# alexklwong/calibrated-backprojection-network

Hardware: AMD Instinct MI355X
Metric: depth-completion frames/sec at 352x1216 (higher is better)
Workload: dtype f32; 1 GPU; KITTI 352x1216, batch 32/GPU, fp32, full KBNet forward in HIP, random xavier weights; frames_per_gpu=32, global_batch=32, height=352, width=1216, n_ranks_seen=1, collective_backend=nccl, gathered_frames=32, launch=HIP graph replay, 2 concurrent sub-batch branch(es)

## Files before the change

calibrated-backprojection-network_amd/csrc/conv1x1s2_split.hip:

```cpp

#include "split_common.h"

namespace kbn {

template <int N, int NBX>
__device__ __forceinline__ void c1_wait_b(f32x4 (&b)[NBX][2]) {
    static_assert(NBX == 1, "one 32-filter block per wave (the 4 x 2 wave form with two was measured and removed)");
    asm volatile("s_waitcnt vmcnt(%2)" : "+v"(b[0][0]), "+v"(b[0][1]) : "n"(N));
}
template <int N>
__device__ __forceinline__ void c1_wait_a(float (&v)[8]) {
    asm volatile("s_waitcnt vmcnt(%8)" : "+v"(v[0]), "+v"(v[1]), "+v"(v[2]), "+v"(v[3]), "+v"(v[4]), "+v"(v[5]), "+v"(v[6]), "+v"(v[7]) : "n"(N));
}

template <int RG, int NB, bool ONE = false>
__global__ __launch_bounds__(SP_THREADS, 1) void conv1x1s2_split_kernel(const SplitConvParams p) {
    constexpr int TH = 8, MB = TH / RG, NT = 128, NPIX = TH * SP_TW;
    static_assert(32 * NB * (8 / RG) == NT, "128 filters per workgroup");
    constexpr int A_PART = 2 * NPIX * 16, A_BYTES = 2 * A_PART;
    constexpr int B_CHUNK = 2 * 2 * NT * 16;
    extern __shared__ __attribute__((aligned(16))) unsigned char smem[];
    asm volatile("s_setreg_imm32_b32 hwreg(HW_REG_MODE, 6, 2), 0");
    const int tid = threadIdx.x, lane = tid & 63;
    const int wave = __builtin_amdgcn_readfirstlane(tid >> 6);
    const int rg = wave % RG, fg = wave / RG;
    const int lm = lane & 31, g = lane >> 5;
    int bid = xcd_remap(blockIdx.x, p.nblocks);
    const int nt = bid % p.nTilesN;
    bid /= p.nTilesN;
    const int tx = bid % p.tilesX;
    bid /= p.tilesX;
    const int ty = bid % p.tilesY;
    const int n = bid / p.tilesY;
    const int oy0 = ty * TH, ox0 = tx * SP_TW;
    const int H = p.H, W = p.W, sH = p.sH, sW = p.sW;
    const long long plane = (long long)sH * sW;
    const int nchunks = p.Cin / SP_CK, last = nchunks - 1;
    float prescale, unscale;
    sp_act_scale(p, n, prescale, unscale);

    const int kg_st = wave >> 2, t256 = tid & 255;
    const int sy = 2 * (oy0 + (t256 >> 5)), sx = 2 * (ox0 + (t256 & 31));
    const int goff = (sy < sH && sx < sW) ? (sy * sW + sx) * 4 : -1;
    const int goff_sub = goff >= 0 ? ((sy >> 1) * W + (sx >> 1)) * 4 : -1;
    const long long plane_sub = (long long)H * W;
    const unsigned char* wp_nt = reinterpret_cast<const unsigned char*>(p.wp) + (long long)nt * nchunks * B_CHUNK;

    float va[2][8];
    auto load_chunk = [&](float (&v)[8], int chunk) {
        int c = chunk * SP_CK, s = 0;
        if (p.nsrc > 1 && c >= p.srcC[0]) { c -= p.srcC[0]; s = 1; }
        const bool sub = p.sub0 && s == 0;
        const long long pl = sub ? plane_sub : plane;
        const float* base = p.src[s] + (long long)n * p.src_bstride[s] + (long long)(c + kg_st * 8) * pl;
        const int go = sub ? goff_sub : goff;
        const unsigned voff = go < 0 ? 0u : (unsigned)go;
#pragma unroll
        for (int k = 0; k < 8; ++k) {
            const float* sb = base + (long long)k * pl;
            asm volatile("global_load_dword %0, %1, %2" : "=v"(v[k]) : "v"(voff), "s"(sb) : "memory");
        }
    };
    auto store_chunk = [&](int buf, const float (&vin)[8]) {
        unsigned char* A = smem + buf * A_BYTES + kg_st * NPIX * 16;
        float v[8];
#pragma unroll
        for (int k = 0; k < 8; ++k) v[k] = goff >= 0 ? vin[k] : 0.f;
        sph8 h1, h2;
        sp_split8(v, prescale, h1, h2);
        *reinterpret_cast<sph8*>(A + t256 * 16) = h1;
        *reinterpret_cast<sph8*>(A + A_PART + t256 * 16) = h2;
    };
    const unsigned boff = (unsigned)((g * NT + fg * 32 * NB + lm) * 16);
    auto load_b = [&](f32x4 (&b)[NB][2], int chunk) {
        const unsigned char* base = wp_nt + (long long)chunk * B_CHUNK;
#pragma unroll
        for (int nb = 0; nb < NB; ++nb)
#pragma unroll
            for (int t = 0; t < 2; ++t) {
                const unsigned char* sb = base + (t * 2 * NT + nb * 32) * 16;
                asm volatile("global_load_dwordx4 %0, %1, %2" : "=v"(b[nb][t]) : "v"(boff), "s"(sb) : "memory");
            }
    };

    spf16 acc[MB][NB], lo[MB][NB];
#pragma unroll
    for (int mb = 0; mb < MB; ++mb)
#pragma unroll
        for (int nb = 0; nb < NB; ++nb)
#pragma unroll
            for (int i = 0; i < 16; ++i) { acc[mb][nb][i] = 0.f; lo[mb][nb][i] = 0.f; }

    const unsigned char* const aptr = smem + (g * NPIX + MB * rg * SP_TW + lm) * 16;
    f32x4 bq[2][NB][2];
    constexpr int NLB = 2 * NB, NLA = 8;
    auto body = [&](int c, auto par_tag) {
        constexpr int PAR = decltype(par_tag)::value;
        load_b(bq[PAR ^ 1], min(c + 1, last));
        load_chunk(va[PAR], min(c + 2, last));
        c1_wait_b<NLA + NLB + NLA>(bq[PAR]);
        if (c <= last) {
            sph8 bw[NB][2], a[MB][2];
#pragma unroll
            for (int nb = 0; nb < NB; ++nb) {
                bw[nb][0] = __builtin_bit_cast(sph8, bq[PAR][nb][0]);
                bw[nb][1] = __builtin_bit_cast(sph8, bq[PAR][nb][1]);
            }
            const int abuf = PAR * A_BYTES;
#pragma unroll
            for (int mb = 0; mb < MB; ++mb)
#pragma unroll
                for (int t = 0; t < 2; ++t) a[mb][t] = *reinterpret_cast<const sph8*>(aptr + abuf + t * A_PART + mb * SP_TW * 16);
            constexpr int TA[3] = {0, 0, 1}, TBP[3] = {0, 1, 0};
#pragma unroll
            for (int t = 0; t < (ONE ? 1 : 3); ++t)
#pragma unroll
                for (int mb = 0; mb < MB; ++mb)
#pragma unroll
                    for (int nb = 0; nb < NB; ++nb) {
                        spf16& d = t > 0 ? lo[mb][nb] : acc[mb][nb];
                        d = __builtin_amdgcn_mfma_f32_32x32x16_f16(a[mb][TA[t]], bw[nb][TBP[t]], d, 0, 0, 0);
                    }
        }
        c1_wait_a<NLB + NLA>(va[PAR ^ 1]);
        store_chunk(PAR ^ 1, va[PAR ^ 1]);
        __syncthreads();
    };

    load_chunk(va[0], 0);
    c1_wait_a<0>(va[0]);
    store_chunk(0, va[0]);
    load_b(bq[0], 0);
    load_chunk(va[1], min(1, last));
    __syncthreads();
    for (int c = 0; c < nchunks; c += 2) {
        body(c, std::integral_constant<int, 0>{});
        body(c + 1, std::integral_constant<int, 1>{});
    }
    asm volatile("s_waitcnt vmcnt(0)" ::: "memory");

    const long long oplane = (long long)H * W;
    float* outn = p.out + (long long)n * p.out_bstride;
    const float* xyzn = p.xyz ? p.xyz + (long long)n * p.xyz_bstride : nullptr;
    const float slope = p.act ? p.slope : 1.f;
    const bool vec4 = p.vec4 != 0;
    float amax = 0.f;
#pragma unroll
    for (int nb = 0; nb < NB; ++nb) {
        const int oc = nt * NT + fg * 32 * NB + nb * 32 + lm;
        const float inv = p.inv_scale[oc] * unscale;
        if (oc >= p.OC) continue;
        float wx[3] = {0.f, 0.f, 0.f};
        if (xyzn) { wx[0] = p.wxyz[oc * 3]; wx[1] = p.wxyz[oc * 3 + 1]; wx[2] = p.wxyz[oc * 3 + 2]; }
#pragma unroll
        for (int mb = 0; mb < MB; ++mb) {
            const int Y = oy0 + MB * rg + mb;
            if (Y >= H) continue;
            float* o = outn + (long long)oc * oplane + (long long)Y * W + ox0 + 4 * g;
#pragma unroll
            for (int q4 = 0; q4 < 4; ++q4) {
                const int X = ox0 + 8 * q4 + 4 * g;
                if (X >= W) continue;
                f32x4 v;
#pragma unroll
                for (int j = 0; j < 4; ++j) {
                    float t = __builtin_fmaf(lo[mb][nb][q4 * 4 + j], 0.00048828125f, acc[mb][nb][q4 * 4 + j]) * inv;
                    if (xyzn && X + j < W) {
                        const float* xp = xyzn + (long long)Y * W + X + j;
                        t += wx[0] * xp[0] + wx[1] * xp[oplane] + wx[2] * xp[2 * oplane];
                    }
                    v[j] = t > 0.f ? t : t * slope;
                }
                if (vec4) {
                    *reinterpret_cast<f32x4*>(o + 8 * q4) = v;
                    amax = sp_amax4(amax, v);
                } else {
#pragma unroll
                    for (int j = 0; j < 4; ++j)
                        if (X + j < W) { o[8 * q4 + j] = v[j]; amax = fmaxf(amax, fin_abs(v[j])); }
                }
            }
        }
    }
    if (p.out_amax) absmax_commit(p.out_amax + n, amax);
}

__global__ void kb_xyz_s2_kernel(const float* __restrict__ depth, long long dbs, int Cd, int H, int W, const float* __restrict__ proj,
                                 const float* __restrict__ kinv, int act, float slope, float* __restrict__ xyz, long long xbs,
                                 int oh, int ow) {
    const int idx = blockIdx.x * blockDim.x + threadIdx.x, n = blockIdx.y;
    if (idx >= oh * ow) return;
    const int oy = idx / ow, ox = idx - oy * ow;
    const int Y = 2 * oy, X = 2 * ox;
    const long long HW = (long long)H * W;
    const float* db = depth + (long long)n * dbs + (long long)Y * W + X;
    float a0 = 0.f, a1 = 0.f, a2 = 0.f, a3 = 0.f;
    int c = 0;
    for (; c + 3 < Cd; c += 4) {
        a0 = fmaf(proj[c], db[(long long)c * HW], a0);
        a1 = fmaf(proj[c + 1], db[(long long)(c + 1) * HW], a1);
        a2 = fmaf(proj[c + 2], db[(long long)(c + 2) * HW], a2);
        a3 = fmaf(proj[c + 3], db[(long long)(c + 3) * HW], a3);
    }
    for (; c < Cd; ++c) a0 = fmaf(proj[c], db[(long long)c * HW], a0);
    const float a = (a0 + a1) + (a2 + a3);
    const float z = act ? leaky_relu(a, slope) : a;
    const float* ki = kinv + (long long)n * 9;
    float* o = xyz + (long long)n * xbs + idx;
#pragma unroll
    for (int j = 0; j < 3; ++j)
        o[(long long)j * oh * ow] = (fmaf(ki[j * 3 + 1], (float)Y, ki[j * 3 + 0] * (float)X) + ki[j * 3 + 2]) * z;
}

__global__ void copy_wxyz_kernel(const float* __restrict__ w, float* __restrict__ wxyz, int OC, int cin_total, int xyz_offset) {
    const int e = blockIdx.x * blockDim.x + threadIdx.x;
    if (e < OC * 3) wxyz[e] = w[(long long)(e / 3) * cin_total + xyz_offset + e % 3];
}

}

extern "C" {

static size_t c1_panel_bytes(int out_channels, int cin) {
    return (size_t)kbn::ceil_div(out_channels, 128) * (128 * 4 + (size_t)(cin / kbn::SP_CK) * (2 * 2 * 128 * 16));
}

size_t kbn_conv1x1s2_split_packed_weight_bytes(int out_channels, int tensor_channels, int has_xyz) {
    if (out_channels < 1 || tensor_channels < 1 || (tensor_channels % kbn::SP_CK) != 0) return 0;
    return c1_panel_bytes(out_channels, tensor_channels) + (has_xyz ? (size_t)out_channels * 3 * 4 : 0);
}

int kbn_conv1x1s2_split_pack_weight(const float* weight, void* packed, int out_channels, int in_channels, int xyz_offset,
                                    kbn_stream_t stream) {
    using namespace kbn;
    const bool has_xyz = xyz_offset >= 0;
    const int cin = in_channels - (has_xyz ? 3 : 0);
    if (!weight || !packed || (has_xyz && xyz_offset > cin) || kbn_conv1x1s2_split_packed_weight_bytes(out_channels, cin, has_xyz) == 0)
        return KBN_ERR_INVALID_ARGUMENT;
    const int ocpad = ceil_div(out_channels, 128) * 128;
    float* inv = static_cast<float*>(packed);
    _Float16* wp = reinterpret_cast<_Float16*>(inv + ocpad);
    const long long total = (long long)((c1_panel_bytes(out_channels, cin) - (size_t)ocpad * 4) / 2);
    split_pack_launch(weight, inv, wp, out_channels, in_channels, cin, 128, total, 1, has_xyz ? xyz_offset : cin, has_xyz ? 3 : 0,
                      (hipStream_t)stream);
    if (has_xyz) {
        float* wxyz = reinterpret_cast<float*>(static_cast<unsigned char*>(packed) + c1_panel_bytes(out_channels, cin));
        hipLaunchKernelGGL(copy_wxyz_kernel, dim3(ceil_div(out_channels * 3, 256)), dim3(256), 0, (hipStream_t)stream, weight, wxyz,
                           out_channels, in_channels, xyz_offset);
    }
    KBN_CHECK_LAUNCH();
    return KBN_OK;
}

int kbn_conv1x1s2_split_forward(const kbn_conv_src* srcs, int n_src, const void* packed_weight, const float* xyz,
                                long long xyz_batch_stride, float* out, long long out_batch_stride, int n, int out_channels,
                                int height, int width, int act_exponent, int apply_activation, float negative_slope,
                                unsigned* out_absmax, kbn_stream_t stream) {
    using namespace kbn;
    if (act_exponent < -60 || act_exponent > 60) return KBN_ERR_INVALID_ARGUMENT;
    if (!srcs || n_src < 1 || n_src > 2 || !packed_weight || !out || n < 1 || out_channels < 1 || height < 1 || width < 1)
        return KBN_ERR_INVALID_ARGUMENT;
    if (knob(KNOB_NO_SPLIT)) return KBN_ERR_UNSUPPORTED;
    SplitConvParams p{};
    int cin = 0;
    for (int s = 0; s < n_src; ++s) {
        const kbn_conv_src& a = srcs[s];
        if (a.kind != KBN_SRC_TENSOR || !a.data || a.channels < 1 || (a.channels % SP_CK) != 0) return KBN_ERR_UNSUPPORTED;
        const bool sub = s == 0 && n_src == 2 && a.src_height == height && a.src_width == width &&
                         (srcs[1].src_height != height || srcs[1].src_width != width);
        if (sub) p.sub0 = 1;
        else {
            if (!p.sH) { p.sH = a.src_height; p.sW = a.src_width; }
            if (a.src_height != p.sH || a.src_width != p.sW) return KBN_ERR_INVALID_ARGUMENT;
        }
        p.src[s] = a.data; p.src_bstride[s] = a.batch_stride; p.srcC[s] = a.channels;
        cin += a.channels;
    }
    if (ceil_div(p.sH, 2) != height || ceil_div(p.sW, 2) != width) return KBN_ERR_INVALID_ARGUMENT;
    if ((long long)p.sH * p.sW > 0x1fffffffLL) return KBN_ERR_UNSUPPORTED;
    if (n_src == 1) { p.src[1] = p.src[0]; p.src_bstride[1] = p.src_bstride[0]; p.srcC[1] = 0; }
    p.nsrc = n_src;
    if (srcs[0].absmax && (n_src == 1 || srcs[1].absmax)) { p.amax[0] = srcs[0].absmax; p.amax[1] = n_src > 1 ? srcs[1].absmax : nullptr; }
    p.out_amax = out_absmax;
    p.nTilesN = ceil_div(out_channels, 128);
    p.inv_scale = static_cast<const float*>(packed_weight);
    p.wp = reinterpret_cast<const _Float16*>(p.inv_scale + p.nTilesN * 128);
    p.xyz = xyz; p.xyz_bstride = xyz_batch_stride;
    p.wxyz = xyz ? reinterpret_cast<const float*>(static_cast<const unsigned char*>(packed_weight) + c1_panel_bytes(out_channels, cin)) : nullptr;
    p.out = out; p.out_bstride = out_batch_stride;
    p.N = n; p.OC = out_channels; p.Cin = cin; p.H = height; p.W = width;
    p.tilesX = ceil_div(width, SP_TW); p.tilesY = ceil_div(height, 8);
    const long long blocks = (long long)p.tilesX * p.tilesY * n * p.nTilesN;
    if (blocks > 0x7fffffffLL) return KBN_ERR_UNSUPPORTED;
    p.nblocks = (int)blocks;
    p.act = apply_activation ? 1 : 0; p.slope = negative_slope;
    p.prescale = ldexpf(1.f, act_exponent); p.unscale = ldexpf(1.f, -act_exponent);
    p.vec4 = !((width & 3) || (reinterpret_cast<uintptr_t>(out) & 15) || (out_batch_stride & 3)) ? 1 : 0;
    if (knob(KNOB_FP16_ONE_TERM))
        hipLaunchKernelGGL((conv1x1s2_split_kernel<2, 1, true>), dim3(p.nblocks), dim3(SP_THREADS), 2 * 2 * 2 * 256 * 16, (hipStream_t)stream, p);
    else hipLaunchKernelGGL((conv1x1s2_split_kernel<2, 1>), dim3(p.nblocks), dim3(SP_THREADS), 2 * 2 * 2 * 256 * 16, (hipStream_t)stream, p);
    KBN_CHECK_LAUNCH();
    return KBN_OK;
}

int kbn_kb_xyz_s2_forward(const float* depth, long long depth_batch_stride, int depth_channels, int height, int width,
                          const float* proj_weight, const float* kinv, int apply_activation, float negative_slope, float* xyz,
                          long long xyz_batch_stride, int n, kbn_stream_t stream) {
    using namespace kbn;
    if (!depth || !proj_weight || !kinv || !xyz || n < 1 || depth_channels < 1 || height < 1 || width < 1) return KBN_ERR_INVALID_ARGUMENT;
    const int oh = ceil_div(height, 2), ow = ceil_div(width, 2);
    hipLaunchKernelGGL(kb_xyz_s2_kernel, dim3(ceil_div(oh * ow, 256), n), dim3(256), 0, (hipStream_t)stream, depth, depth_batch_stride,
                       depth_channels, height, width, proj_weight, kinv, apply_activation ? 1 : 0, negative_slope, xyz,
                       xyz_batch_stride, oh, ow);
    KBN_CHECK_LAUNCH();
    return KBN_OK;
}

}
```

calibrated-backprojection-network_amd/ops.py:

```python

from __future__ import annotations

import contextlib
import ctypes as C
import functools
from typing import List, Optional, Sequence

import torch

from . import _lib
from ._lib import ConvSrc, KbnError, check


def _stream() -> int:
    return torch.cuda.current_stream().cuda_stream


def _on_tensor_device(fn):
    @functools.wraps(fn)
    def wrapper(*args, **kwargs):
        idx = None
        for a in list(args) + list(kwargs.values()):
            if isinstance(a, torch.Tensor) and a.is_cuda:
                if idx is None:
# ... 615 lines not shown


@_on_tensor_device
def pack_conv3x3_split_weight(weight: torch.Tensor, out: Optional[torch.Tensor] = None, stride: int = 1,
                              folded_up2x: bool = False, transposed: bool = False) -> torch.Tensor:
    mode = 4 if transposed else (3 if folded_up2x else (2 if stride == 2 else 0))
    lib = _lib.load()
    w = _weight(_deconv_weight(weight) if transposed else weight)
    oc, cin, kh, kw = w.shape
    nbytes = lib.kbn_conv3x3_split_packed_weight_bytes(oc, cin, mode) if (kh, kw) == (3, 3) else 0
    if nbytes == 0:
        raise KbnError(f"conv3x3_split needs a 3x3 weight with in_channels % 16 == 0, got {tuple(w.shape)}")
    return _pack_into(out, nbytes, w, lambda p: lib.kbn_conv3x3_split_pack_weight(w.data_ptr(), p, oc, cin, mode, _stream()),
                      "kbn_conv3x3_split_pack_weight")


def act_exponent_for(amax: float) -> int:
    import struct
    b = struct.unpack("<I", struct.pack("<f", abs(amax)))[0] if amax == amax else 0x7fc00000
    return max(-100, min(100, 14 + 127 - (b >> 23)))


def conv3x3_split_executed_flops(n, cin, out_channels, height, width, stride=1, folded_up2x=False):
    if folded_up2x:
        nblk = 16 if (out_channels <= 16 and cin % 32 == 0) else 32
        seg = 16 if nblk == 16 else 32
        sh, sw = height // 2, width // 2
        wide = out_channels >= 64 and (-(-out_channels // 32)) % 2 == 0
        if nblk == 32 and wide and sw >= 32 and 1 <= sw % 32 <= 16:
            px = sh * 32 * (sw // 32) + -(-sh // 2) * 32
        else:
            px = sh * (-(-sw // seg) * seg)
        return 3 * 2.0 * n * px * cin * 16 * (-(-out_channels // nblk) * nblk)
    if stride == 1 and width >= 32 and 1 <= width % 32 <= 16:
        px = height * 32 * (width // 32) + -(-height // 2) * 32
    else:
        px = height * (-(-width // 32) * 32)
    return 3 * 2.0 * n * px * cin * 9 * (-(-out_channels // 32) * 32)


@_on_tensor_device
def conv3x3_split(srcs: List[ConvSrc], packed_weight: torch.Tensor, n: int, out_channels: int, height: int, width: int,
                  out: torch.Tensor, up2x: bool = False, negative_slope: Optional[float] = 0.2, stride: int = 1,
                  act_exponent: int = -6, folded_up2x: bool = False, out_absmax: Optional[torch.Tensor] = None,
                  transposed: bool = False, ksplit: int = 1):
    if transposed and not (up2x and folded_up2x):
        raise KbnError("conv3x3_split: transposed goes with up2x and folded_up2x")
    if up2x and stride != 1:
        raise KbnError("conv3x3_split: up2x and stride 2 are mutually exclusive")
    lib = _lib.load()
    arr = (ConvSrc * len(srcs))(*srcs)
    pair = isinstance(out, PairTensor)
    if pair:
        optr, obs = (None, 0) if (out.sub is None or stride != 2) else _planes(out.sub, "out.sub")
        if out_absmax is None:
            out_absmax = out.absmax
    else:
        optr, obs = _planes(out, "out")
    want = (n, 16 if (pair and up2x and folded_up2x and out_channels <= 16) else out_channels, height, width)
    if tuple(out.shape) != want:
        raise KbnError(f"out has shape {tuple(out.shape)}, expected {want}")
    cin = sum(s.channels for s in srcs)
    flops = 2.0 * n * height * width * cin * 9 * out_channels / (4 if transposed else 1)
    mode = (4 if transposed else (3 if folded_up2x else 1)) if up2x else (2 if stride == 2 else 0)
    if ksplit > 1:
        if pair or mode == 1:
            raise KbnError("conv3x3_split: ksplit goes with the plain / stride-2 / folded up-conv forms and an fp32 output")
        ws = torch.empty((ksplit, n, out_channels, height, width), device=out.device, dtype=torch.float32)
        done = _launched("kbn_conv3x3_split_forward_ksplit", ("conv_split", "", "conv_split_s2", "conv_split_upfold", "conv_split_upfold")[mode], flops,
                         lambda: lib.kbn_conv3x3_split_forward_ksplit(arr, len(srcs), packed_weight.data_ptr(), optr, obs, n, out_channels, height, width,
                                                                      mode, max(-60, min(60, int(act_exponent))), *_act_args(negative_slope),
                                                                      _slot_ptr(out_absmax, n), int(ksplit), ws.data_ptr(), _stream()),
                         executed=conv3x3_split_executed_flops(n, cin, out_channels, height, width, stride, up2x and folded_up2x),
                         pipe="fp16", nbytes=_src_bytes(srcs, n) + 4.0 * n * height * width * out_channels * (1 + 2 * ksplit))
        return out if done else None
    if not _launched("kbn_conv3x3_split_forward", ("conv_split", "conv_split_up", "conv_split_s2", "conv_split_upfold", "conv_split_upfold")[mode], flops,
                     lambda: lib.kbn_conv3x3_split_forward(arr, len(srcs), packed_weight.data_ptr(), optr, obs, n,
                                                           out_channels, height, width,
                                                           mode, max(-60, min(60, int(act_exponent))),
                                                           *_act_args(negative_slope), _slot_ptr(out_absmax, n),
                                                           out.data.data_ptr() if pair else None,
                                                           out.data.stride(0) if pair else 0,
                                                           out.scale.data_ptr() if pair else None, _stream()),
                     executed=conv3x3_split_executed_flops(n, cin, out_channels, height, width, stride, up2x and folded_up2x),
                     pipe="fp16", nbytes=_src_bytes(srcs, n) + 4.0 * n * height * width * want[1]
                     + (4.0 * n * out_channels * out.sub.shape[2] * out.sub.shape[3] if (pair and out.sub is not None and stride == 2) else 0.0)):
        return None
    return out


def ksplit_for(cin: int, out_channels: int, height: int, width: int, stride: int = 1, cus: int = 256, up2x: bool = False, frames: int = 1) -> int:
    if up2x:
        tiles = -(-(width // 2) // 32) * (-(-(height // 2) // 8)) * (-(-out_channels // 64))
    else:
        tiles = -(-width // 32) * (-(-height // (8 if stride == 2 else 16))) * (-(-out_channels // (128 if stride == 2 else 64)))
    tiles *= max(1, int(frames))
    chunks = cin // 16
    if tiles * 2 > cus or chunks < 4 or 4 * out_channels * height * width * max(1, int(frames)) > (16 << 20):
        return 1
    ks = min(16, chunks // 2, max(1, cus // tiles))
    while ks > 1 and -(-chunks // ks) * (ks - 1) >= chunks:
        ks -= 1
    return ks


@_on_tensor_device
def pack_conv1x1s2_split_weight(weight: torch.Tensor, xyz_offset: int = -1, out: Optional[torch.Tensor] = None) -> torch.Tensor:
    lib = _lib.load()
    w = _weight(weight)
    oc, cin, kh, kw = w.shape
    has_xyz = xyz_offset >= 0
    nbytes = lib.kbn_conv1x1s2_split_packed_weight_bytes(oc, cin - (3 if has_xyz else 0), 1 if has_xyz else 0) if (kh, kw) == (1, 1) else 0
    if nbytes == 0:
        raise KbnError(f"conv1x1s2_split needs a 1x1 weight with tensor channels % 16 == 0, got {tuple(w.shape)}")
    return _pack_into(out, nbytes, w, lambda p: lib.kbn_conv1x1s2_split_pack_weight(w.data_ptr(), p, oc, cin, int(xyz_offset), _stream()),
                      "kbn_conv1x1s2_split_pack_weight")


@_on_tensor_device
def kb_xyz_s2(depth: torch.Tensor, proj_weight: torch.Tensor, kinv: torch.Tensor, negative_slope: Optional[float] = 0.2,
              out: Optional[torch.Tensor] = None) -> torch.Tensor:
    lib = _lib.load()
    dptr, dbs = _planes(depth, "depth")
    n, cd, h, w = depth.shape
    oh, ow = (h + 1) // 2, (w + 1) // 2
    pw = proj_weight.detach().contiguous()
    if pw.numel() != cd or tuple(kinv.shape) != (n, 3, 3) or not kinv.is_contiguous():
        raise KbnError("kb_xyz_s2: proj_weight must hold one weight per depth channel, kinv must be a dense N x 3 x 3")
    if out is None:
        out = torch.empty((n, 3, oh, ow), device=depth.device, dtype=torch.float32)
    optr, obs = _planes(out, "xyz")
    check(_launch("kb_xyz", 2.0 * n * oh * ow * cd,
                  lambda: lib.kbn_kb_xyz_s2_forward(dptr, dbs, cd, h, w, pw.data_ptr(), kinv.data_ptr(), *_act_args(negative_slope),
                                                    optr, obs, n, _stream()), nbytes=4.0 * n * oh * ow * (cd + 3)), "kbn_kb_xyz_s2_forward")
    return out


@_on_tensor_device
def conv1x1s2_split(srcs: List[ConvSrc], packed_weight: torch.Tensor, xyz: Optional[torch.Tensor], n: int, out_channels: int,
                    height: int, width: int, out: torch.Tensor, negative_slope: Optional[float] = 0.2, act_exponent: int = -6,
                    out_absmax: Optional[torch.Tensor] = None):
    lib = _lib.load()
    arr = (ConvSrc * len(srcs))(*srcs)
    optr, obs = _planes(out, "out")
    if tuple(out.shape) != (n, out_channels, height, width):
        raise KbnError(f"out has shape {tuple(out.shape)}, expected {(n, out_channels, height, width)}")
    xptr, xbs = (None, 0)
    if xyz is not None:
        if tuple(xyz.shape) != (n, 3, height, width):
            raise KbnError(f"xyz has shape {tuple(xyz.shape)}, expected {(n, 3, height, width)}")
        xptr, xbs = _planes(xyz, "xyz")
    cin = sum(s.channels for s in srcs)
    flops = 2.0 * n * height * width * (cin + (3 if xyz is not None else 0)) * out_channels
    executed = 3 * 2.0 * n * (-(-height // 8) * 8) * (-(-width // 32) * 32) * cin * (-(-out_channels // 128) * 128)
    if not _launched("kbn_conv1x1s2_split_forward", "conv_split_1x1s2", flops,
                     lambda: lib.kbn_conv1x1s2_split_forward(arr, len(srcs), packed_weight.data_ptr(), xptr, xbs, optr, obs, n,
                                                             out_channels, height, width, max(-60, min(60, int(act_exponent))),
                                                             *_act_args(negative_slope), _slot_ptr(out_absmax, n), _stream()),
                     executed=executed, pipe="fp16",
                     nbytes=4.0 * n * height * width * (cin + (3 if xyz is not None else 0) + out_channels)):
        return None
    return out


@_on_tensor_device
def pack_kb1_front_weight(w_conv0: torch.Tensor, w_conv_image: torch.Tensor, w_conv_fused: torch.Tensor,
                          out: Optional[torch.Tensor] = None) -> Optional[torch.Tensor]:
    lib = _lib.load()
    w0, wi, wf = _weight(w_conv0, "w_conv0"), _weight(w_conv_image, "w_conv_image"), _weight(w_conv_fused, "w_conv_fused")
    f0, c = w0.shape[0], w0.shape[1]
    fi = wi.shape[0]
    if tuple(w0.shape[2:]) != (3, 3) or tuple(wi.shape) != (fi, f0, 3, 3) or tuple(wf.shape) != (fi, f0 + 3, 1, 1):
        return None
    nbytes = lib.kbn_kb1_front_packed_weight_bytes(c, f0, fi)
    if nbytes == 0:
        return None
    return _pack_into(out, nbytes, w0, lambda p: lib.kbn_kb1_front_pack_weight(w0.data_ptr(), wi.data_ptr(), wf.data_ptr(), p, c, f0, fi, _stream()),
                      "kbn_kb1_front_pack_weight")


def kb1_front_supported(image_channels: int, conv0_filters: int, kb_filters: int, height: int, width: int,
                        conv0_negative_slope: float, depth_branch: bool = False) -> bool:
    lib = _lib.load()
    q = lib.kbn_kb1_depth_front_query if depth_branch else lib.kbn_kb1_front_query
    return q(int(image_channels), int(conv0_filters), int(kb_filters), int(height), int(width), float(conv0_negative_slope)) == _lib.KBN_OK


@_on_tensor_device
def pack_kb1_front_next_weight(w_conv_fused: torch.Tensor, image_channels: int, out: Optional[torch.Tensor] = None) -> Optional[torch.Tensor]:
    lib = _lib.load()
    wf = _weight(w_conv_fused, "w_conv_fused")
    fo, cin = wf.shape[0], wf.shape[1]
    cf = cin - 3 - image_channels
    if tuple(wf.shape[2:]) != (1, 1) or cf < 0:
        return None
    nbytes = lib.kbn_kb1_front_next_packed_weight_bytes(int(image_channels), int(cf), int(fo))
    if nbytes == 0:
        return None
    return _pack_into(out, nbytes, wf, lambda p: lib.kbn_kb1_front_next_pack_weight(wf.data_ptr(), p, int(image_channels), int(cf), int(fo), _stream()),
                      "kbn_kb1_front_next_pack_weight")


def kb1_front_next_supported(image_channels: int, conv0_filters: int, kb_filters: int, next_filters: int, height: int, width: int,
                             conv0_negative_slope: float) -> bool:
    return _lib.load().kbn_kb1_front_next_query(int(image_channels), int(conv0_filters), int(kb_filters), int(next_filters), int(height),
                                                int(width), float(conv0_negative_slope)) == _lib.KBN_OK


@_on_tensor_device
def kb1_front(image: torch.Tensor, packed_weight: torch.Tensor, xyz: Optional[torch.Tensor],
              conv0_filters: int, kb_filters: int, out_image: torch.Tensor, out_fused: torch.Tensor,
              conv0_negative_slope: float = 0.2, kb_negative_slope: float = 0.2, out_image_absmax=None, out_fused_absmax=None,
              next_fused=None):
    lib = _lib.load()
    iptr, ibs = _planes(image, "image")
    n, c, h, w = image.shape
    oh, ow = (h + 1) // 2, (w + 1) // 2
    for t, nm in ((out_image, "out_image"), (out_fused, "out_fused")):
        if tuple(t.shape) != (n, kb_filters, oh, ow):
            raise KbnError(f"{nm} has shape {tuple(t.shape)}, expected {(n, kb_filters, oh, ow)}")
    oi, oibs = _planes(out_image, "out_image")
    of, ofbs = _planes(out_fused, "out_fused")
    xptr, xbs = (None, 0)
    if xyz is not None:
        if tuple(xyz.shape) != (n, 3, oh, ow):
            raise KbnError(f"xyz has shape {tuple(xyz.shape)}, expected {(n, 3, oh, ow)}")
        xptr, xbs = _planes(xyz, "xyz")
    flops = 2.0 * n * (h * w * c * 9 * conv0_filters + oh * ow * conv0_filters * 9 * kb_filters + oh * ow * (conv0_filters + 3) * kb_filters)
    tiles = n * (-(-oh // 8)) * (-(-ow // 16))
    executed = tiles * (conv0_filters // 16) * (36 * 9 + 8 * 6 * (kb_filters // 16) * 3) * 2.0 * 16 * 16 * 32
    nbytes = 4.0 * n * (h * w * c + oh * ow * (2 * kb_filters + (3 if xyz is not None else 0)))
    if next_fused is None:
        call = lambda: lib.kbn_kb1_front_forward(iptr, ibs, packed_weight.data_ptr(), xptr, xbs,
                                                 oi, oibs, of, ofbs, n, c, conv0_filters, kb_filters, h, w,
                                                 float(conv0_negative_slope), float(kb_negative_slope),
                                                 _slot_ptr(out_image_absmax, n), _slot_ptr(out_fused_absmax, n), _stream())
    else:
        packed_next, xyz_next, out_next, slope_next, amax_next = next_fused
        h2, w2 = (oh + 1) // 2, (ow + 1) // 2
        fo = out_next.shape[1]
        if tuple(out_next.shape) != (n, fo, h2, w2) or tuple(xyz_next.shape) != (n, 3, h2, w2):
            raise KbnError(f"next_fused: out {tuple(out_next.shape)} / xyz {tuple(xyz_next.shape)}, expected {(n, fo, h2, w2)} / {(n, 3, h2, w2)}")
        on, onbs = _planes(out_next, "out_next_fused")
        xn, xnbs = _planes(xyz_next, "xyz_next")
        flops += 2.0 * n * h2 * w2 * (2 * kb_filters + 3) * fo
        executed += tiles * 2 * (fo // 16) * (2 * kb_filters // 32) * 3 * 2.0 * 16 * 16 * 32
        nbytes += 4.0 * n * h2 * w2 * (fo + 3)
        call = lambda: lib.kbn_kb1_front_next_forward(iptr, ibs, packed_weight.data_ptr(), xptr, xbs,
                                                      oi, oibs, of, ofbs, n, c, conv0_filters, kb_filters, h, w,
                                                      float(conv0_negative_slope), float(kb_negative_slope),
                                                      _slot_ptr(out_image_absmax, n), _slot_ptr(out_fused_absmax, n),
                                                      packed_next.data_ptr(), xn, xnbs, on, onbs, fo, float(slope_next),
                                                      _slot_ptr(amax_next, n), _stream())
    if not _launched("kbn_kb1_front_forward", "kb1_front", flops, call, executed=executed, pipe="fp16", nbytes=nbytes):
        return None
    return out_image, out_fused


@_on_tensor_device
def pack_kb1_depth_front_weight(w_conv0: torch.Tensor, w_conv_depth: torch.Tensor, w_proj: torch.Tensor,
                                out: Optional[torch.Tensor] = None) -> Optional[torch.Tensor]:
    lib = _lib.load()
    w0, wc, wp = _weight(w_conv0, "w_conv0"), _weight(w_conv_depth, "w_conv_depth"), _weight(w_proj, "w_proj")
    f0, c = w0.shape[0], w0.shape[1]
    fd = wc.shape[0]
    if tuple(w0.shape[2:]) != (3, 3) or tuple(wc.shape) != (fd, f0 + 3, 3, 3) or wp.numel() != f0:
        return None
    nbytes = lib.kbn_kb1_depth_front_packed_weight_bytes(c, f0, fd)
    if nbytes == 0:
        return None
    return _pack_into(out, nbytes, w0, lambda p: lib.kbn_kb1_depth_front_pack_weight(w0.data_ptr(), wc.data_ptr(), wp.data_ptr(), p, c, f0, fd, _stream()),
                      "kbn_kb1_depth_front_pack_weight")


@_on_tensor_device
def kb1_depth_front(depth: torch.Tensor, kinv: torch.Tensor, packed_weight: torch.Tensor, conv0_filters: int, kb_filters: int,
                    out_depth: torch.Tensor, conv0_negative_slope: float = 0.2, kb_negative_slope: float = 0.2,
                    proj_negative_slope: Optional[float] = 0.2, out_depth_absmax=None, xyz: Optional[torch.Tensor] = None):
    lib = _lib.load()
    dptr, dbs = _planes(depth, "depth")
    n, c, h, w = depth.shape
    oh, ow = (h + 1) // 2, (w + 1) // 2
    if tuple(out_depth.shape) != (n, kb_filters, oh, ow):
        raise KbnError(f"out_depth has shape {tuple(out_depth.shape)}, expected {(n, kb_filters, oh, ow)}")
    if tuple(kinv.shape) != (n, 3, 3) or not kinv.is_contiguous():
        raise KbnError("kinv must be a dense N x 3 x 3")
    _require(kinv, "kinv", 3)
    if xyz is None:
        xyz = torch.empty((n, 3, oh, ow), device=depth.device, dtype=torch.float32)
    optr, obs = _planes(out_depth, "out_depth")
    xptr, xbs = _planes(xyz, "xyz")
    flops = 2.0 * n * (h * w * c * 9 * conv0_filters + oh * ow * ((conv0_filters + 3) * 9 * kb_filters + conv0_filters))
    tiles = n * (-(-oh // 8)) * (-(-ow // 16))
    executed = tiles * (36 * 9 + 8 * 15) * 2.0 * 16 * 16 * 32
    if not _launched("kbn_kb1_depth_front_forward", "kb1_depth_front", flops,
                     lambda: lib.kbn_kb1_depth_front_forward(dptr, dbs, kinv.data_ptr(), packed_weight.data_ptr(), optr, obs, xptr, xbs,
                                                             n, c, conv0_filters, kb_filters, h, w, float(conv0_negative_slope),
                                                             float(kb_negative_slope), *_act_args(proj_negative_slope),
                                                             _slot_ptr(out_depth_absmax, n), _stream()),
                     executed=executed, pipe="fp16", nbytes=4.0 * n * (h * w * c + oh * ow * (kb_filters + 3))):
        return None
    return out_depth, xyz


@_on_tensor_device
def pack_s2d_depth_front_weight(w_pool_convs: List[torch.Tensor], w_conv: torch.Tensor, out: Optional[torch.Tensor] = None) -> Optional[torch.Tensor]:
    lib = _lib.load()
# ... 286 lines not shown
```

Before: 2980 frames/s.

## Halve conv1x1s2 tile height, deepen activation prefetch ring, raise occupancy

The strided 1x1 split-fp16 conv kernel now uses 4-row output tiles instead of 8, so each wave keeps two accumulator pairs instead of four. Launch bounds allow 4 workgroups per CU. Activation staging is spread over all 512 threads, each loading 4 channels. The activation prefetch ring grows from 2 to 4 chunks in flight. The aim is more latency hiding through occupancy and deeper prefetch, at the cost of twice as many workgroups, each re-reading the weight panel, and more per-thread prefetch registers.

New measurement: 2998 frames/s, median of 6. No clear change (+0.6%).

```diff
diff --git a/calibrated-backprojection-network_amd/csrc/conv1x1s2_split.hip b/calibrated-backprojection-network_amd/csrc/conv1x1s2_split.hip
--- a/calibrated-backprojection-network_amd/csrc/conv1x1s2_split.hip
+++ b/calibrated-backprojection-network_amd/csrc/conv1x1s2_split.hip
@@ -3,22 +3,39 @@
 
 namespace kbn {
 
-template <int N, int NBX>
-__device__ __forceinline__ void c1_wait_b(f32x4 (&b)[NBX][2]) {
-    static_assert(NBX == 1, "one 32-filter block per wave (the 4 x 2 wave form with two was measured and removed)");
-    asm volatile("s_waitcnt vmcnt(%2)" : "+v"(b[0][0]), "+v"(b[0][1]) : "n"(N));
-}
+constexpr int C1_TH = 4, C1_NT = 128, C1_RING = 4;
+constexpr int C1_LDS = 2 * 2 * 2 * C1_TH * SP_TW * 16;
+
 template <int N>
-__device__ __forceinline__ void c1_wait_a(float (&v)[8]) {
-    asm volatile("s_waitcnt vmcnt(%8)" : "+v"(v[0]), "+v"(v[1]), "+v"(v[2]), "+v"(v[3]), "+v"(v[4]), "+v"(v[5]), "+v"(v[6]), "+v"(v[7]) : "n"(N));
-}
-
-template <int RG, int NB, bool ONE = false>
-__global__ __launch_bounds__(SP_THREADS, 1) void conv1x1s2_split_kernel(const SplitConvParams p) {
-    constexpr int TH = 8, MB = TH / RG, NT = 128, NPIX = TH * SP_TW;
-    static_assert(32 * NB * (8 / RG) == NT, "128 filters per workgroup");
+__device__ __forceinline__ void c1_wait_b(f32x4 (&b)[2]) {
+    asm volatile("s_waitcnt vmcnt(%2)" : "+v"(b[0]), "+v"(b[1]) : "n"(N));
+}
+template <int N>
+__device__ __forceinline__ void c1_wait_a(float (&v)[4]) {
+    asm volatile("s_waitcnt vmcnt(%4)" : "+v"(v[0]), "+v"(v[1]), "+v"(v[2]), "+v"(v[3]) : "n"(N));
+}
+__device__ __forceinline__ void c1_split4(const float (&v)[4], float prescale, sph4& h1, sph4& h2) {
+    const float prescale_hi = prescale * 2048.f;
+#pragma unroll
+    for (int k = 0; k < 4; k += 2) {
+        const f32x2 a = {v[k], v[k + 1]};
+        const sph2 c1 = __builtin_convertvector(a * prescale, sph2);
+        const f32x2 f = {(float)c1[0], (float)c1[1]};
+        const f32x2 hi = a * prescale_hi;
+        const f32x2 r = {__builtin_fmaf(f[0], -2048.f, hi[0]), __builtin_fmaf(f[1], -2048.f, hi[1])};
+        const sph2 c2 = __builtin_convertvector(r, sph2);
+        h1[k] = c1[0]; h1[k + 1] = c1[1];
+        h2[k] = c2[0]; h2[k + 1] = c2[1];
+    }
+}
+
+template <bool ONE = false>
+__global__ __launch_bounds__(SP_THREADS, 4) void conv1x1s2_split_kernel(const SplitConvParams p) {
+    constexpr int TH = C1_TH, MB = 2, RG = TH / MB, NT = C1_NT, NPIX = TH * SP_TW, D = C1_RING;
+    static_assert(32 * (8 / RG) == NT && NPIX * 4 == SP_THREADS, "8 waves: 2 row groups x 4 filter blocks; 4 staging threads per pixel");
     constexpr int A_PART = 2 * NPIX * 16, A_BYTES = 2 * A_PART;
     constexpr int B_CHUNK = 2 * 2 * NT * 16;
+    static_assert(2 * A_BYTES == C1_LDS, "launch size");
     extern __shared__ __attribute__((aligned(16))) unsigned char smem[];
     asm volatile("s_setreg_imm32_b32 hwreg(HW_REG_MODE, 6, 2), 0");
     const int tid = threadIdx.x, lane = tid & 63;
@@ -39,73 +56,65 @@
     float prescale, unscale;
     sp_act_scale(p, n, prescale, unscale);
 
-    const int kg_st = wave >> 2, t256 = tid & 255;
-    const int sy = 2 * (oy0 + (t256 >> 5)), sx = 2 * (ox0 + (t256 & 31));
+    const int kg_st = wave >> 2, hf_st = (wave >> 1) & 1, pix = tid & (NPIX - 1);
+    const int sy = 2 * (oy0 + (pix >> 5)), sx = 2 * (ox0 + (pix & 31));
     const int goff = (sy < sH && sx < sW) ? (sy * sW + sx) * 4 : -1;
     const int goff_sub = goff >= 0 ? ((sy >> 1) * W + (sx >> 1)) * 4 : -1;
     const long long plane_sub = (long long)H * W;
     const unsigned char* wp_nt = reinterpret_cast<const unsigned char*>(p.wp) + (long long)nt * nchunks * B_CHUNK;
 
-    float va[2][8];
-    auto load_chunk = [&](float (&v)[8], int chunk) {
+    float va[D][4];
+    auto load_chunk = [&](float (&v)[4], int chunk) {
         int c = chunk * SP_CK, s = 0;
         if (p.nsrc > 1 && c >= p.srcC[0]) { c -= p.srcC[0]; s = 1; }
         const bool sub = p.sub0 && s == 0;
         const long long pl = sub ? plane_sub : plane;
-        const float* base = p.src[s] + (long long)n * p.src_bstride[s] + (long long)(c + kg_st * 8) * pl;
+        const float* base = p.src[s] + (long long)n * p.src_bstride[s] + (long long)(c + kg_st * 8 + hf_st * 4) * pl;
         const int go = sub ? goff_sub : goff;
         const unsigned voff = go < 0 ? 0u : (unsigned)go;
 #pragma unroll
-        for (int k = 0; k < 8; ++k) {
+        for (int k = 0; k < 4; ++k) {
             const float* sb = base + (long long)k * pl;
             asm volatile("global_load_dword %0, %1, %2" : "=v"(v[k]) : "v"(voff), "s"(sb) : "memory");
         }
     };
-    auto store_chunk = [&](int buf, const float (&vin)[8]) {
-        unsigned char* A = smem + buf * A_BYTES + kg_st * NPIX * 16;
-        float v[8];
-#pragma unroll
-        for (int k = 0; k < 8; ++k) v[k] = goff >= 0 ? vin[k] : 0.f;
-        sph8 h1, h2;
-        sp_split8(v, prescale, h1, h2);
-        *reinterpret_cast<sph8*>(A + t256 * 16) = h1;
-        *reinterpret_cast<sph8*>(A + A_PART + t256 * 16) = h2;
+    auto store_chunk = [&](int buf, const float (&vin)[4]) {
+        unsigned char* A = smem + buf * A_BYTES + (kg_st * NPIX + pix) * 16 + hf_st * 8;
+        float v[4];
+#pragma unroll
+        for (int k = 0; k < 4; ++k) v[k] = goff >= 0 ? vin[k] : 0.f;
+        sph4 h1, h2;
+        c1_split4(v, prescale, h1, h2);
+        *reinterpret_cast<sph4*>(A) = h1;
+        *reinterpret_cast<sph4*>(A + A_PART) = h2;
     };
-    const unsigned boff = (unsigned)((g * NT + fg * 32 * NB + lm) * 16);
-    auto load_b = [&](f32x4 (&b)[NB][2], int chunk) {
+    const unsigned boff = (unsigned)((g * NT + fg * 32 + lm) * 16);
+    auto load_b = [&](f32x4 (&b)[2], int chunk) {
         const unsigned char* base = wp_nt + (long long)chunk * B_CHUNK;
 #pragma unroll
-        for (int nb = 0; nb < NB; ++nb)
-#pragma unroll
-            for (int t = 0; t < 2; ++t) {
-                const unsigned char* sb = base + (t * 2 * NT + nb * 32) * 16;
-                asm volatile("global_load_dwordx4 %0, %1, %2" : "=v"(b[nb][t]) : "v"(boff), "s"(sb) : "memory");
-            }
+        for (int t = 0; t < 2; ++t) {
+            const unsigned char* sb = base + t * 2 * NT * 16;
+            asm volatile("global_load_dwordx4 %0, %1, %2" : "=v"(b[t]) : "v"(boff), "s"(sb) : "memory");
+        }
     };
 
-    spf16 acc[MB][NB], lo[MB][NB];
+    spf16 acc[MB], lo[MB];
 #pragma unroll
     for (int mb = 0; mb < MB; ++mb)
 #pragma unroll
-        for (int nb = 0; nb < NB; ++nb)
-#pragma unroll
-            for (int i = 0; i < 16; ++i) { acc[mb][nb][i] = 0.f; lo[mb][nb][i] = 0.f; }
+        for (int i = 0; i < 16; ++i) { acc[mb][i] = 0.f; lo[mb][i] = 0.f; }
 
     const unsigned char* const aptr = smem + (g * NPIX + MB * rg * SP_TW + lm) * 16;
-    f32x4 bq[2][NB][2];
-    constexpr int NLB = 2 * NB, NLA = 8;
-    auto body = [&](int c, auto par_tag) {
-        constexpr int PAR = decltype(par_tag)::value;
+    f32x4 bq[2][2];
+    constexpr int NLB = 2, NLA = 4;
+    auto body = [&](int c, auto j_tag) {
+        constexpr int J = decltype(j_tag)::value, PAR = J & 1;
         load_b(bq[PAR ^ 1], min(c + 1, last));
-        load_chunk(va[PAR], min(c + 2, last));
+        load_chunk(va[J], min(c + D, last));
         c1_wait_b<NLA + NLB + NLA>(bq[PAR]);
         if (c <= last) {
-            sph8 bw[NB][2], a[MB][2];
-#pragma unroll
-            for (int nb = 0; nb < NB; ++nb) {
-                bw[nb][0] = __builtin_bit_cast(sph8, bq[PAR][nb][0]);
-                bw[nb][1] = __builtin_bit_cast(sph8, bq[PAR][nb][1]);
-            }
+            const sph8 bw[2] = {__builtin_bit_cast(sph8, bq[PAR][0]), __builtin_bit_cast(sph8, bq[PAR][1])};
+            sph8 a[MB][2];
             const int abuf = PAR * A_BYTES;
 #pragma unroll
             for (int mb = 0; mb < MB; ++mb)
@@ -115,27 +124,29 @@
 #pragma unroll
             for (int t = 0; t < (ONE ? 1 : 3); ++t)
 #pragma unroll
-                for (int mb = 0; mb < MB; ++mb)
-#pragma unroll
-                    for (int nb = 0; nb < NB; ++nb) {
-                        spf16& d = t > 0 ? lo[mb][nb] : acc[mb][nb];
-                        d = __builtin_amdgcn_mfma_f32_32x32x16_f16(a[mb][TA[t]], bw[nb][TBP[t]], d, 0, 0, 0);
-                    }
-        }
-        c1_wait_a<NLB + NLA>(va[PAR ^ 1]);
-        store_chunk(PAR ^ 1, va[PAR ^ 1]);
+                for (int mb = 0; mb < MB; ++mb) {
+                    spf16& d = t > 0 ? lo[mb] : acc[mb];
+                    d = __builtin_amdgcn_mfma_f32_32x32x16_f16(a[mb][TA[t]], bw[TBP[t]], d, 0, 0, 0);
+                }
+        }
+        c1_wait_a<(D - 1) * (NLB + NLA)>(va[(J + 1) % D]);
+        store_chunk(PAR ^ 1, va[(J + 1) % D]);
         __syncthreads();
     };
 
+    static_assert(D == 4, "the loop below holds D copies of the body; D even (weight set and A buffer go by parity)");
     load_chunk(va[0], 0);
     c1_wait_a<0>(va[0]);
     store_chunk(0, va[0]);
     load_b(bq[0], 0);
-    load_chunk(va[1], min(1, last));
+#pragma unroll
+    for (int j = 1; j < D; ++j) load_chunk(va[j], min(j, last));
     __syncthreads();
-    for (int c = 0; c < nchunks; c += 2) {
+    for (int c = 0; c < nchunks; c += D) {
         body(c, std::integral_constant<int, 0>{});
         body(c + 1, std::integral_constant<int, 1>{});
+        body(c + 2, std::integral_constant<int, 2>{});
+        body(c + 3, std::integral_constant<int, 3>{});
     }
     asm volatile("s_waitcnt vmcnt(0)" ::: "memory");
 
@@ -145,11 +156,9 @@
     const float slope = p.act ? p.slope : 1.f;
     const bool vec4 = p.vec4 != 0;
     float amax = 0.f;
-#pragma unroll
-    for (int nb = 0; nb < NB; ++nb) {
-        const int oc = nt * NT + fg * 32 * NB + nb * 32 + lm;
-        const float inv = p.inv_scale[oc] * unscale;
-        if (oc >= p.OC) continue;
+    const int oc = nt * NT + fg * 32 + lm;
+    const float inv = p.inv_scale[oc] * unscale;
+    if (oc < p.OC) {
         float wx[3] = {0.f, 0.f, 0.f};
         if (xyzn) { wx[0] = p.wxyz[oc * 3]; wx[1] = p.wxyz[oc * 3 + 1]; wx[2] = p.wxyz[oc * 3 + 2]; }
 #pragma unroll
@@ -164,7 +173,7 @@
                 f32x4 v;
 #pragma unroll
                 for (int j = 0; j < 4; ++j) {
-                    float t = __builtin_fmaf(lo[mb][nb][q4 * 4 + j], 0.00048828125f, acc[mb][nb][q4 * 4 + j]) * inv;
+                    float t = __builtin_fmaf(lo[mb][q4 * 4 + j], 0.00048828125f, acc[mb][q4 * 4 + j]) * inv;
                     if (xyzn && X + j < W) {
                         const float* xp = xyzn + (long long)Y * W + X + j;
                         t += wx[0] * xp[0] + wx[1] * xp[oplane] + wx[2] * xp[2 * oplane];
@@ -289,7 +298,7 @@
     p.wxyz = xyz ? reinterpret_cast<const float*>(static_cast<const unsigned char*>(packed_weight) + c1_panel_bytes(out_channels, cin)) : nullptr;
     p.out = out; p.out_bstride = out_batch_stride;
     p.N = n; p.OC = out_channels; p.Cin = cin; p.H = height; p.W = width;
-    p.tilesX = ceil_div(width, SP_TW); p.tilesY = ceil_div(height, 8);
+    p.tilesX = ceil_div(width, SP_TW); p.tilesY = ceil_div(height, C1_TH);
     const long long blocks = (long long)p.tilesX * p.tilesY * n * p.nTilesN;
     if (blocks > 0x7fffffffLL) return KBN_ERR_UNSUPPORTED;
     p.nblocks = (int)blocks;
@@ -297,8 +306,8 @@
     p.prescale = ldexpf(1.f, act_exponent); p.unscale = ldexpf(1.f, -act_exponent);
     p.vec4 = !((width & 3) || (reinterpret_cast<uintptr_t>(out) & 15) || (out_batch_stride & 3)) ? 1 : 0;
     if (knob(KNOB_FP16_ONE_TERM))
-        hipLaunchKernelGGL((conv1x1s2_split_kernel<2, 1, true>), dim3(p.nblocks), dim3(SP_THREADS), 2 * 2 * 2 * 256 * 16, (hipStream_t)stream, p);
-    else hipLaunchKernelGGL((conv1x1s2_split_kernel<2, 1>), dim3(p.nblocks), dim3(SP_THREADS), 2 * 2 * 2 * 256 * 16, (hipStream_t)stream, p);
+        hipLaunchKernelGGL((conv1x1s2_split_kernel<true>), dim3(p.nblocks), dim3(SP_THREADS), C1_LDS, (hipStream_t)stream, p);
+    else hipLaunchKernelGGL((conv1x1s2_split_kernel<false>), dim3(p.nblocks), dim3(SP_THREADS), C1_LDS, (hipStream_t)stream, p);
     KBN_CHECK_LAUNCH();
     return KBN_OK;
 }
diff --git a/calibrated-backprojection-network_amd/ops.py b/calibrated-backprojection-network_amd/ops.py
--- a/calibrated-backprojection-network_amd/ops.py
+++ b/calibrated-backprojection-network_amd/ops.py
@@ -791,7 +791,7 @@
         xptr, xbs = _planes(xyz, "xyz")
     cin = sum(s.channels for s in srcs)
     flops = 2.0 * n * height * width * (cin + (3 if xyz is not None else 0)) * out_channels
-    executed = 3 * 2.0 * n * (-(-height // 8) * 8) * (-(-width // 32) * 32) * cin * (-(-out_channels // 128) * 128)
+    executed = 3 * 2.0 * n * (-(-height // 4) * 4) * (-(-width // 32) * 32) * cin * (-(-out_channels // 128) * 128)
     if not _launched("kbn_conv1x1s2_split_forward", "conv_split_1x1s2", flops,
                      lambda: lib.kbn_conv1x1s2_split_forward(arr, len(srcs), packed_weight.data_ptr(), xptr, xbs, optr, obs, n,
                                                              out_channels, height, width, max(-60, min(60, int(act_exponent))),
```
